# microsoft/tf2-gnn

Measured on NVIDIA H100. Metric: edges/sec (fused gather-msg-scatter), higher is better.
Workload: dtype f32

## Files before the change

### tf2_gnn_b200/csrc/fused_rgcn.cu

```cuda
#include <cuda.h>

#include <algorithm>
#include <cstdio>
#include <cstdlib>
#include <mutex>
#include <vector>

#include "gemm.cuh"
#include "wgmma_tile.cuh"

namespace tfgnn {

constexpr int kFuBM = 128;
constexpr int kFuBK = 32;
constexpr int kFuATileBytes = kFuBM * kFuBK * 4;
constexpr int kFuGatherWarps = 8;
constexpr int kFuFirstGatherWarp = 9;
constexpr int kFuThreads = 32 * (kFuFirstGatherWarp + kFuGatherWarps);
constexpr int kFuMaxSlots = 8;
constexpr int kFuMaxBN = 64;
constexpr int kFuSmemLimit = 227 * 1024;
constexpr int kFuMaxQ = 8;

struct FusedParams {
// ... 90 lines not shown
    ids = ids0B;
    in_blk = 0;
    i_blk = i_pos;
    ids_next = load_ids(i_blk + 32);
    ids0B = load_ids(__shfl_sync(0xffffffffu, rpB, 0));
  }
  template <int NV, int QT = 0, bool FULL = false>
  __device__ __forceinline__ void issue() {
    const int Qc = QT > 0 ? QT : Q;
    while (i_pos == i_end && ic + 1 < ncalls) next_call();
    if (i_pos < i_end) {
      if (in_blk == 32) {
        in_blk = 0;
        i_blk += 32;
        ids = ids_next;
        ids_next = load_ids(i_blk + 32);
      }
      const int s = __shfl_sync(0xffffffffu, ids, in_blk);
      const float* rowp = h + (long long)s * ldh;
#pragma unroll
      for (int j = 0; j < NV; ++j)
        if (FULL || lane + 32 * j < C4) ptx::cp_async16(ibuf + 512u * j, rowp + 128 * j);
      ++in_blk;
      ++i_pos;
    }
    ptx::cp_async_commit();
    if (++islot == Qc) {
      islot = 0;
      ibuf = buf_s;
    } else {
      ibuf += row_bytes;
    }
  }
};

__device__ __forceinline__ void cp_async_wait_oldest(int Q) {
  switch (Q) {
    case 1: asm volatile("cp.async.wait_group 0;" ::: "memory"); break;
    case 2: asm volatile("cp.async.wait_group 1;" ::: "memory"); break;
    case 3: asm volatile("cp.async.wait_group 2;" ::: "memory"); break;
    case 4: asm volatile("cp.async.wait_group 3;" ::: "memory"); break;
    case 5: asm volatile("cp.async.wait_group 4;" ::: "memory"); break;
    case 6: asm volatile("cp.async.wait_group 5;" ::: "memory"); break;
    case 7: asm volatile("cp.async.wait_group 6;" ::: "memory"); break;
    default: asm volatile("cp.async.wait_group 7;" ::: "memory"); break;
  }
}

template <int NV, int QT = 0, bool FULL = false>
__device__ __forceinline__ void gather_warp_main(const FusedParams& p, int lane, int gw, int Q_in, uint8_t* bufs,
                                                 long long unit0, long long unit_step, long long total_units,
                                                 int ctas, int rank, int tile_rows, int row_off, int w_row0, int rpw,
                                                 int ring_row0, uint64_t* slot_ready, uint64_t* slot_free, int split,
                                                 int split_rank, uint32_t peer_slot_ready0) {
  const int Q = QT > 0 ? QT : Q_in;
  const int D = p.D, C4 = p.D >> 2, normalize = p.normalize;
  const bool no_store = p.debug_skip & 16;
  const int kFuSlots = p.num_slots;
  float* const ring = p.ring;
  const uint64_t pol_keep = ptx::policy_evict_last();
  const long long my_units = unit0 < total_units ? (total_units - unit0 + unit_step - 1) / unit_step : 0;
  GatherIssue g;
  g.row_ptr = p.row_ptr; g.src = p.src; g.h = p.h + 4 * lane; g.M = p.M; g.V = p.V; g.L = p.L; g.ldh = p.ldh;
  g.skip = p.debug_skip & 1; g.C4 = C4;
  g.lane = lane; g.gw = gw; g.Q = Q; g.ncalls = (int)(my_units * p.L);
  g.unit0 = unit0; g.unit_step = unit_step; g.ctas = ctas; g.rank = rank;
  g.tile_rows = tile_rows; g.rpw = rpw; g.row_off = row_off; g.w_row0 = w_row0;
  g.buf_s = ptx::smem_u32(bufs) + (uint32_t)lane * 16u;
  g.row_bytes = (uint32_t)p.D * 4;
  g.ic = 0; g.islot = 0; g.in_blk = 0; g.ibuf = g.buf_s;
  g.rpA = g.rp_of(0); g.rpB = g.rp_of(1); g.rpC = g.rp_of(2);
  g.i_pos = __shfl_sync(0xffffffffu, g.rpA, 0);
  g.i_end = __shfl_sync(0xffffffffu, g.rpA, g.nrows_of(0));
  g.i_blk = g.i_pos;
  g.ids = g.load_ids(g.i_blk);
  g.ids_next = g.load_ids(g.i_blk + 32);
  g.ids0B = g.load_ids(__shfl_sync(0xffffffffu, g.rpB, 0));
  int crp = g.rpA, crp_next = g.rpB;
  int cslot = 0;
  uint32_t cbuf = g.buf_s;
  for (int i = 0; i < Q; ++i) g.template issue<NV, QT, FULL>();

  float4 acc[NV];
#pragma unroll
  for (int j = 0; j < NV; ++j) acc[j] = make_float4(0.f, 0.f, 0.f, 0.f);

  for (int cc = 0; cc < g.ncalls; ++cc) {
    int l, v0, nrows;
    g.call_rows(cc, l, v0, nrows);
    const int rp = crp;
    crp = crp_next;
    crp_next = g.rp_of(cc + 2);
    const int slot = cc % kFuSlots;
    if (split) ptx::mbar_wait_cluster(&slot_free[slot], ((cc / kFuSlots) & 1) ^ 1);
    else ptx::mbar_wait_backoff(&slot_free[slot], ((cc / kFuSlots) & 1) ^ 1, p.sleep_long);
    float* dst = ring + ((size_t)ring_row0 + (size_t)slot * tile_rows + (size_t)row_off + (size_t)w_row0) * D + 4 * lane;
    int row = 0;
    int seg_begin = __shfl_sync(0xffffffffu, rp, 0);
    int seg_end = __shfl_sync(0xffffffffu, rp, 1);
    const int e_end = __shfl_sync(0xffffffffu, rp, nrows);
    auto flush = [&]() {
      const float scale = normalize ? 1.0f / ((float)(seg_end - seg_begin) + kSmallNumber) : 1.0f;
#pragma unroll
      for (int j = 0; j < NV; ++j) {
        if (lane + 32 * j < C4 && !no_store)
          ptx::st_f4_hint(dst + 128 * j,
                          make_float4(acc[j].x * scale, acc[j].y * scale, acc[j].z * scale, acc[j].w * scale),
                          pol_keep);
        acc[j] = make_float4(0.f, 0.f, 0.f, 0.f);
      }
      dst += D;
      ++row;
      seg_begin = seg_end;
      seg_end = __shfl_sync(0xffffffffu, rp, row + 1);
    };
    for (int e = seg_begin; e < e_end; ++e) {
      while (e >= seg_end) flush();
      cp_async_wait_oldest(Q);
#pragma unroll
      for (int j = 0; j < NV; ++j) {
        if (FULL || lane + 32 * j < C4) {
          const float4 x = ptx::lds_f4(cbuf + 512u * j);
          acc[j].x += x.x; acc[j].y += x.y; acc[j].z += x.z; acc[j].w += x.w;
        }
      }
      if (++cslot == Q) {
        cslot = 0;
        cbuf = g.buf_s;
      } else {
        cbuf += g.row_bytes;
      }
      g.template issue<NV, QT, FULL>();
    }
    while (row < nrows) flush();
    asm volatile("fence.proxy.async.global;" ::: "memory");
    __syncwarp();
    if (lane == 0) {
      if (split) {
        ptx::mbar_arrive_cluster_release(ptx::mapa_shared(ptx::smem_u32(&slot_ready[slot]), (uint32_t)split_rank));
        ptx::mbar_arrive_cluster_release(peer_slot_ready0 + (uint32_t)slot * 8u);
      } else {
        ptx::mbar_arrive(&slot_ready[slot]);
      }
    }
  }
  asm volatile("cp.async.wait_group 0;" ::: "memory");
}

template <int BN, bool FOLDED = false>
__device__ __forceinline__ void fused_epilogue(const FusedParams& p, const HalfTileAcc<BN>& c, long long m0, int n0, int cw,
                                               int t) {
  const int w = t >> 5, lane = t & 31, cq = 2 * (lane & 3);
  const uint64_t pol_stream = ptx::policy_evict_first();
  const bool ln = p.epi.ln_gamma != nullptr;
#pragma unroll
  for (int h = 0; h < 2; ++h) {
    const long long row = m0 + 64 * cw + 16 * w + (lane >> 2) + 8 * h;
    const bool row_ok = row < p.V;
    float v[BN / 4];
    if (FOLDED) {
#pragma unroll
      for (int i = 0; i < BN / 8; ++i) {
        v[2 * i] = c.main[4 * i + 2 * h];
        v[2 * i + 1] = c.main[4 * i + 2 * h + 1];
      }
    } else {
      acc_row<BN>(c, h, v);
    }
    if (p.epi.row_norm && row_ok) {
      const float inv_rn = 1.0f / fu_row_norm(p.epi, row);
#pragma unroll
      for (int j = 0; j < BN / 4; ++j) v[j] *= inv_rn;
    }
    if (p.epi.bias) {
#pragma unroll
      for (int i = 0; i < BN / 8; ++i) {
        const float2 b = __ldg(reinterpret_cast<const float2*>(p.epi.bias + n0 + 8 * i + cq));
        v[2 * i] += b.x; v[2 * i + 1] += b.y;
      }
    }
    apply_act_vec<BN / 4>(v, p.epi.act);
    if (ln) {
      float s1 = 0.f;
#pragma unroll
      for (int j = 0; j < BN / 4; ++j) s1 += v[j];
      s1 += __shfl_xor_sync(0xffffffffu, s1, 1);
      s1 += __shfl_xor_sync(0xffffffffu, s1, 2);
      const float mean = s1 / (float)BN;
      float s2 = 0.f;
#pragma unroll
      for (int j = 0; j < BN / 4; ++j) { const float d = v[j] - mean; s2 = fmaf(d, d, s2); }
      s2 += __shfl_xor_sync(0xffffffffu, s2, 1);
      s2 += __shfl_xor_sync(0xffffffffu, s2, 2);
      const float rstd = rsqrtf(s2 / (float)BN + p.epi.ln_eps);
#pragma unroll
      for (int i = 0; i < BN / 8; ++i) {
        const float2 g = __ldg(reinterpret_cast<const float2*>(p.epi.ln_gamma + n0 + 8 * i + cq));
        const float2 b = __ldg(reinterpret_cast<const float2*>(p.epi.ln_beta + n0 + 8 * i + cq));
        v[2 * i] = (v[2 * i] - mean) * rstd * g.x + b.x;
        v[2 * i + 1] = (v[2 * i + 1] - mean) * rstd * g.y + b.y;
      }
    }
    if (!row_ok) continue;
#pragma unroll
    for (int i = 0; i < BN / 8; ++i) {
      const long long off = row * p.ldc + n0 + 8 * i + cq;
      const float2 val = make_float2(v[2 * i], v[2 * i + 1]);
      if (p.C_mc) {
        asm volatile("multimem.st.relaxed.sys.global.v2.f32 [%0], {%1, %2};" ::"l"(p.C_mc + off), "f"(val.x), "f"(val.y)
                     : "memory");
      } else {
        asm volatile("st.global.L2::cache_hint.v2.f32 [%0], {%1, %2}, %3;" ::"l"(p.C + off), "f"(val.x), "f"(val.y),
                     "l"(pol_stream)
                     : "memory");
        for (int pr = 0; pr < p.n_peer; ++pr) *reinterpret_cast<float2*>(p.C_peer[pr] + off) = val;
      }
    }
  }
}

template <int NV, int BN>
__global__ void __launch_bounds__(kFuThreads, 1)
fused_rgcn_kernel(const __grid_constant__ CUtensorMap map_a, const __grid_constant__ CUtensorMap map_b,
                  const FusedParams p) {
  extern __shared__ uint8_t smem_raw[];
  uint8_t* smem = reinterpret_cast<uint8_t*>((reinterpret_cast<uintptr_t>(smem_raw) + 1023) & ~uintptr_t(1023));
  constexpr int b_tile_bytes = BN * kFuBK * 4;
  constexpr int stage_bytes = 2 * kFuATileBytes + 2 * b_tile_bytes;
  const int S = p.num_stages;
  const bool split = p.split != 0;
  uint64_t* bars = reinterpret_cast<uint64_t*>(smem + (size_t)S * stage_bytes);
  uint64_t* full = bars;
  uint64_t* empty = bars + S;
  uint64_t* slot_ready = bars + 2 * S;
  uint64_t* slot_free = bars + 2 * S + kFuMaxSlots;
  uint8_t* gbuf = reinterpret_cast<uint8_t*>(
      (reinterpret_cast<uintptr_t>(bars + 2 * S + 2 * kFuMaxSlots) + 127) & ~uintptr_t(127));

  const int warp = threadIdx.x >> 5, lane = threadIdx.x & 31, wg = warp >> 2;
  const uint32_t srank = split ? ptx::cluster_ctarank() : 0u;
  const int kClu = split ? 2 : 1;
  const long long total_units = p.m_tiles;
  const long long unit0 = blockIdx.x / kClu, unit_step = gridDim.x / kClu;
  const int n_pass = p.n_tiles;
  const int kFuSlots = p.num_slots;

  if (threadIdx.x == 0) {
    ptx::prefetch_tensormap(&map_a);
    ptx::prefetch_tensormap(&map_b);
    for (int s = 0; s < S; ++s) {
      ptx::mbar_init(&full[s], 1);
      ptx::mbar_init(&empty[s], 2);
    }
    for (int r = 0; r < kFuMaxSlots; ++r) {
      ptx::mbar_init(&slot_ready[r], kFuGatherWarps * (split ? 2 : 1));
      ptx::mbar_init(&slot_free[r], 2 * (split ? 2 : 1));
    }
    ptx::fence_barrier_init();
  }
  __syncthreads();
  if (split) ptx::cluster_sync_all();
  const int ring_row0 = (split ? blockIdx.x / 2 : blockIdx.x) * kFuSlots * kFuBM;
  const uint32_t peer_slot_ready0 = split ? ptx::mapa_shared(ptx::smem_u32(&slot_ready[0]), srank ^ 1u) : 0u;
  const uint32_t peer_slot_free0 = split ? ptx::mapa_shared(ptx::smem_u32(&slot_free[0]), srank ^ 1u) : 0u;

  if (warp == 8) {
    if (lane == 0) {
      uint32_t it = 0, slot_it = 0;
      const uint64_t pol_keep = ptx::policy_evict_last();
      for (long long unit = unit0; unit < total_units; unit += unit_step, slot_it += p.L) {
        for (int pass = 0; pass < n_pass; ++pass) {
          const int n0 = (int)srank * p.cta_n + pass * BN;
          for (int l = 0; l < p.L; ++l) {
            const uint32_t sq = slot_it + l;
            const int slot = sq % kFuSlots;
            if (split) ptx::mbar_wait_cluster(&slot_ready[slot], (sq / kFuSlots) & 1);
            else ptx::mbar_wait_backoff(&slot_ready[slot], (sq / kFuSlots) & 1, p.sleep_long);
            for (int kb = 0; kb < p.kb_per_type; ++kb, ++it) {
              const int s = it % S;
              const uint32_t ph = (it / S) & 1;
              ptx::mbar_wait_backoff(&empty[s], ph ^ 1, p.sleep_crit);
              uint8_t* st = smem + (size_t)s * stage_bytes;
              ptx::mbar_arrive_expect_tx(&full[s], kFuATileBytes + 2 * b_tile_bytes);
              ptx::tma_load_2d_hint(st, &map_a, &full[s], kb * kFuBK, ring_row0 + slot * kFuBM, pol_keep);
              const int kcol = (l * p.kb_per_type + kb) * kFuBK;
              ptx::tma_load_2d_hint(st + 2 * kFuATileBytes, &map_b, &full[s], kcol, n0, pol_keep);
              ptx::tma_load_2d_hint(st + 2 * kFuATileBytes + b_tile_bytes, &map_b, &full[s], kcol, p.N + n0, pol_keep);
            }
          }
        }
      }
    }
  } else if (wg < 2) {
    const int cw = wg, t = threadIdx.x & 127;
    HalfTileAcc<BN> c;
    uint32_t it = 0, slot_base_it = 0;
    for (long long unit = unit0; unit < total_units; unit += unit_step, slot_base_it += p.L) {
      for (int pass = 0; pass < n_pass; ++pass) {
        int prev_s = 0;
        bool first = true;
        for (int l = 0; l < p.L; ++l) {
          const uint32_t slot_it = slot_base_it + l;
          for (int kb = 0; kb < p.kb_per_type; ++kb, ++it) {
            const int s = it % S;
            const uint32_t ph = (it / S) & 1;
            ptx::mbar_wait_backoff(&full[s], ph, p.sleep_crit);
            const bool slot_done = kb == p.kb_per_type - 1 && pass == n_pass - 1;
            if (slot_done && p.discard_ring && !split) {
              const char* sb = reinterpret_cast<const char*>(
                  p.ring + ((size_t)ring_row0 + (size_t)(slot_it % kFuSlots) * kFuBM + (size_t)cw * 64) * p.D);
              const int lines = 64 * p.D * 4 / 128;
              for (int i = t; i < lines; i += 128) ptx::discard_l2_128(sb + (size_t)i * 128);
            }
            const uint32_t st = ptx::smem_u32(smem + (size_t)s * stage_bytes);
            split_a_half<128>(st, cw, t, p.corr_bf16);
            ptx::fence_proxy_async_smem();
            ptx::warpgroup_sync(1 + cw);
            if (slot_done && t == 0) {
              ptx::mbar_arrive(&slot_free[slot_it % kFuSlots]);
              if (split) ptx::mbar_arrive_cluster_release(peer_slot_free0 + (uint32_t)(slot_it % kFuSlots) * 8u);
            }
            ptx::wgmma_fence();
            mma_kblock<BN, 128>(c, st, st + 2 * kFuATileBytes, cw, p.corr_bf16, first);
            ptx::wgmma_commit();
            ptx::wgmma_wait<1>();
            if (!first && t == 0) ptx::mbar_arrive(&empty[prev_s]);
            prev_s = s;
            first = false;
          }
        }
        ptx::wgmma_wait<0>();
        fence_acc<BN>(c);
        if (t == 0) ptx::mbar_arrive(&empty[prev_s]);
        fused_epilogue<BN>(p, c, unit * kFuBM, (int)srank * p.cta_n + pass * BN, cw, t);
      }
    }
  } else {
    const int gw = warp - kFuFirstGatherWarp;
    uint8_t* my_bufs = gbuf + (size_t)gw * p.gather_q * ((size_t)p.D * 4);
    const int rpw = split ? kFuBM / 2 / kFuGatherWarps : kFuBM / kFuGatherWarps;
    const int row_off = split ? (int)srank * (kFuBM / 2) : 0;
#define TFGNN_FU_GATHER(QT, FULL)                                                                                     \
    gather_warp_main<NV, QT, FULL>(p, lane, gw, p.gather_q, my_bufs, unit0, unit_step, total_units, 1, 0, kFuBM,       \
                                   row_off, gw * rpw, rpw, ring_row0, slot_ready, slot_free, split ? 1 : 0, (int)srank, \
                                   peer_slot_ready0)
    if (p.gather_q == kFuMaxQ && p.D == 128 * NV) TFGNN_FU_GATHER(kFuMaxQ, true);
    else TFGNN_FU_GATHER(0, false);
#undef TFGNN_FU_GATHER
  }

  if (split) {
    __syncwarp();
    ptx::cluster_sync_all();
  }
}

constexpr int kRtBM = 64;
constexpr int kRtATileBytes = kRtBM * kFuBK * 4;
constexpr int kRtGatherWarps = 7;
constexpr int kRtFirstGatherWarp = 9;
constexpr int kRtThreads = 512;
constexpr int kRtMaxH = 256;
constexpr uint32_t kRtConsumerRegs = 184;
constexpr uint32_t kRtOtherRegs = 72;

template <int NV, int BN>
__global__ void __launch_bounds__(kRtThreads, 1)
fused_rgcn_rows_kernel(const __grid_constant__ CUtensorMap map_a, const __grid_constant__ CUtensorMap map_b,
                       const FusedParams p) {
  extern __shared__ uint8_t smem_raw[];
  uint8_t* smem = reinterpret_cast<uint8_t*>((reinterpret_cast<uintptr_t>(smem_raw) + 1023) & ~uintptr_t(1023));
  constexpr int H = 2 * BN;
  constexpr int w_tile_bytes = H * kFuBK * 4;
  constexpr int stage_bytes = 2 * kRtATileBytes + 2 * w_tile_bytes;
  const int S = p.num_stages;
  uint64_t* bars = reinterpret_cast<uint64_t*>(smem + (size_t)S * stage_bytes);
  uint64_t* full = bars;
  uint64_t* empty = bars + S;
  uint64_t* slot_ready = bars + 2 * S;
  uint64_t* slot_free = bars + 2 * S + kFuMaxSlots;
  uint8_t* gbuf = reinterpret_cast<uint8_t*>(
      (reinterpret_cast<uintptr_t>(bars + 2 * S + 2 * kFuMaxSlots) + 127) & ~uintptr_t(127));

  const int warp = threadIdx.x >> 5, lane = threadIdx.x & 31, wg = warp >> 2;
  const uint32_t srank = ptx::cluster_ctarank();
  const long long total_units = (p.m_tiles + 1) / 2;
  const long long unit0 = blockIdx.x / 2, unit_step = gridDim.x / 2;
  const int kSlots = p.num_slots;

  if (threadIdx.x == 0) {
    ptx::prefetch_tensormap(&map_a);
    ptx::prefetch_tensormap(&map_b);
    for (int s = 0; s < S; ++s) {
      ptx::mbar_init(&full[s], 1);
      ptx::mbar_init(&empty[s], 4);
    }
    for (int r = 0; r < kFuMaxSlots; ++r) {
      ptx::mbar_init(&slot_ready[r], kRtGatherWarps);
      ptx::mbar_init(&slot_free[r], 2);
    }
    ptx::fence_barrier_init();
  }
  __syncthreads();
  ptx::cluster_sync_all();
  const int ring_row0 = blockIdx.x * kSlots * kRtBM;

  if (wg >= 2) {
    ptx::setmaxnreg_dec<kRtOtherRegs>();
    if (warp == 8) {
      if (lane == 0) {
        uint32_t it = 0, slot_it = 0;
        const uint64_t pol_keep = ptx::policy_evict_last();
        for (long long unit = unit0; unit < total_units; unit += unit_step, slot_it += p.L) {
          for (int l = 0; l < p.L; ++l) {
            const uint32_t sq = slot_it + l;
            const int slot = sq % kSlots;
            ptx::mbar_wait_backoff(&slot_ready[slot], (sq / kSlots) & 1, p.sleep_long);
            for (int kb = 0; kb < p.kb_per_type; ++kb, ++it) {
              const int s = it % S;
              const uint32_t ph = (it / S) & 1;
              ptx::mbar_wait_cluster(&empty[s], ph ^ 1);
              uint8_t* st = smem + (size_t)s * stage_bytes;
              ptx::mbar_arrive_expect_tx(&full[s], kRtATileBytes + 2 * w_tile_bytes);
              ptx::tma_load_2d_hint(st, &map_a, &full[s], kb * kFuBK, ring_row0 + slot * kRtBM, pol_keep);
              const int kcol = (l * p.kb_per_type + kb) * kFuBK;
              ptx::tma_load_2d_multicast_hint(st + 2 * kRtATileBytes + (int)srank * w_tile_bytes, &map_b, &full[s], kcol,
                                              (int)srank * H, (uint16_t)0x3, pol_keep);
            }
          }
        }
      }
    } else {
      const int gw = warp - kRtFirstGatherWarp;
      const int w_row0 = kRtBM * gw / kRtGatherWarps, rpw = kRtBM * (gw + 1) / kRtGatherWarps - w_row0;
      uint8_t* my_bufs = gbuf + (size_t)gw * p.gather_q * ((size_t)p.D * 4);
#define TFGNN_RT_GATHER(QT, FULL)                                                                                      \
      gather_warp_main<NV, QT, FULL>(p, lane, gw, p.gather_q, my_bufs, unit0, unit_step, total_units, 2, (int)srank,   \
                                     kRtBM, 0, w_row0, rpw, ring_row0, slot_ready, slot_free, 0, 0, 0u)
      if (p.gather_q == kFuMaxQ && p.D == 128 * NV) TFGNN_RT_GATHER(kFuMaxQ, true);
      else TFGNN_RT_GATHER(0, false);
#undef TFGNN_RT_GATHER
    }
  } else {
    ptx::setmaxnreg_inc<kRtConsumerRegs>();
    const int cw = wg, t = threadIdx.x & 127;
    const uint32_t empty0_cta0 = ptx::mapa_shared(ptx::smem_u32(&empty[0]), 0u);
    const uint32_t empty0_cta1 = ptx::mapa_shared(ptx::smem_u32(&empty[0]), 1u);
    auto release_stage = [&](int s) {
      if (t == 0) {
        ptx::mbar_arrive_cluster_release(empty0_cta0 + (uint32_t)s * 8u);
        ptx::mbar_arrive_cluster_release(empty0_cta1 + (uint32_t)s * 8u);
      }
    };
    HalfTileAcc<BN> c;
    uint32_t it = 0, slot_base_it = 0;
    for (long long unit = unit0; unit < total_units; unit += unit_step, slot_base_it += p.L) {
      bool first = true;
      for (int l = 0; l < p.L; ++l) {
        const int slot = (slot_base_it + l) % kSlots;
        for (int kb = 0; kb < p.kb_per_type; ++kb, ++it) {
          const int s = it % S;
          const uint32_t ph = (it / S) & 1;
          ptx::mbar_wait_backoff(&full[s], ph, p.sleep_crit);
          const bool slot_done = kb == p.kb_per_type - 1;
          if (slot_done && p.discard_ring) {
            const char* sb = reinterpret_cast<const char*>(
                p.ring + ((size_t)ring_row0 + (size_t)slot * kRtBM + (size_t)cw * (kRtBM / 2)) * p.D);
            const int lines = kRtBM / 2 * p.D * 4 / 128;
            for (int i = t; i < lines; i += 128) ptx::discard_l2_128(sb + (size_t)i * 128);
          }
          const uint32_t st = ptx::smem_u32(smem + (size_t)s * stage_bytes);
          split_a_half<128, kRtBM>(st, cw, t, p.corr_bf16);
          ptx::fence_proxy_async_smem();
          ptx::warpgroup_pair_sync(1);
          if (slot_done && t == 0) ptx::mbar_arrive(&slot_free[slot]);
          const uint32_t w = st + 2 * kRtATileBytes + (uint32_t)(cw * BN * 128);
          ptx::wgmma_fence();
          mma_kblock_at<BN, 128>(c, st, st + kRtATileBytes, w, w + w_tile_bytes, p.corr_bf16, first);
          ptx::wgmma_commit();
          ptx::wgmma_wait<0>();
          release_stage(s);
          first = false;
        }
      }
      fence_acc<BN>(c);
#pragma unroll
      for (int j = 0; j < BN / 2; ++j) c.main[j] += c.corr[j];
      fused_epilogue<BN, true>(p, c, (2 * unit + srank) * kRtBM, cw * BN, 0, t);
    }
  }
  __syncwarp();
  ptx::cluster_sync_all();
}

typedef CUresult (*EncodeTiledFn)(CUtensorMap*, CUtensorMapDataType, cuuint32_t, void*, const cuuint64_t*,
                                  const cuuint64_t*, const cuuint32_t*, const cuuint32_t*, CUtensorMapInterleave,
                                  CUtensorMapSwizzle, CUtensorMapL2promotion, CUtensorMapFloatOOBfill);
static EncodeTiledFn fu_encode_fn() {
  static EncodeTiledFn fn = nullptr;
  static std::once_flag once;
  std::call_once(once, [] {
    void* p = nullptr;
    cudaDriverEntryPointQueryResult qres;
    if (cudaGetDriverEntryPoint("cuTensorMapEncodeTiled", &p, cudaEnableDefault, &qres) == cudaSuccess &&
        qres == cudaDriverEntryPointSuccess)
      fn = reinterpret_cast<EncodeTiledFn>(p);
  });
  return fn;
}

static int fused_block_n(int n) {
  for (int bn = kFuMaxBN; bn >= 16; bn -= 16)
    if (n % bn == 0) return bn;
  return 0;
}

bool fused_rgcn_supported(long long V, int L, int D, int H, const float* h, const float* out, int ldo) {
  if (V < 1 || L < 1 || D % 32 != 0 || D > 512 || H % 16 != 0 || H < 16 || H > 512) return false;
  if (fused_block_n(H) < H && L + 1 > kFuMaxSlots) return false;
  if ((reinterpret_cast<uintptr_t>(h) | reinterpret_cast<uintptr_t>(out)) & 15) return false;
  if (ldo % 4 != 0) return false;
  return gemm_tc_supported(V, H, L * D, h, D, out, ldo) && fu_encode_fn() != nullptr;
}

bool fused_rgcn_ln_supported(int H) { return H <= kFuMaxBN; }

static std::mutex g_l2_mu;
static int g_l2_want_mb = -1;
static bool g_l2_set[64] = {};
static size_t g_l2_saved[64] = {};

int set_l2_persist_mb(int mb) {
  std::lock_guard<std::mutex> lock(g_l2_mu);
  g_l2_want_mb = mb;
  for (bool& b : g_l2_set) b = false;
  return 0;
}

static size_t g_l2_effective[64] = {};

static int ensure_l2_persist_carveout(size_t need_bytes) {
  int dev = 0;
  TFGNN_CUDA(cudaGetDevice(&dev));
  if (dev < 0 || dev >= 64) return 0;
  std::lock_guard<std::mutex> lock(g_l2_mu);
  long long want_mb = g_l2_want_mb;
  if (want_mb < 0) {
    static const int env_mb = [] { const char* e = getenv("TFGNN_B200_L2_PERSIST_MB"); return e ? atoi(e) : -1; }();
    want_mb = env_mb;
  }
  size_t want = want_mb >= 0 ? (size_t)want_mb << 20 : std::max((size_t)72 << 20, need_bytes + ((size_t)4 << 20));
  if (g_l2_set[dev] && (want_mb >= 0 || g_l2_effective[dev] >= want)) return 0;
  g_l2_set[dev] = true;
  if (want == 0) return 0;
  int max_persist = 0;
  if (cudaDeviceGetAttribute(&max_persist, cudaDevAttrMaxPersistingL2CacheSize, dev) != cudaSuccess || max_persist <= 0) {
    cudaGetLastError();
    return 0;
  }
  if (want > (size_t)max_persist) want = (size_t)max_persist;
  size_t cur = 0;
  if (cudaDeviceGetLimit(&cur, cudaLimitPersistingL2CacheSize) != cudaSuccess) { cudaGetLastError(); return 0; }
  g_l2_effective[dev] = cur;
  if (cur >= want) {
    if (want == (size_t)max_persist) g_l2_effective[dev] = (size_t)-1;
    return 0;
  }
  if (!g_l2_saved[dev]) g_l2_saved[dev] = cur + 1;
  cudaDeviceSetLimit(cudaLimitPersistingL2CacheSize, want);
  cudaGetLastError();
  g_l2_effective[dev] = want == (size_t)max_persist ? (size_t)-1 : want;
  return 0;
}

void restore_l2_persist_carveout() {
  std::lock_guard<std::mutex> lock(g_l2_mu);
  int cur_dev = 0;
  if (cudaGetDevice(&cur_dev) != cudaSuccess) { cudaGetLastError(); return; }
  for (int d = 0; d < 64; ++d) {
    if (!g_l2_saved[d]) continue;
    if (cudaSetDevice(d) == cudaSuccess) cudaDeviceSetLimit(cudaLimitPersistingL2CacheSize, g_l2_saved[d] - 1);
    g_l2_saved[d] = 0;
    g_l2_set[d] = false;
    g_l2_effective[d] = 0;
  }
  cudaSetDevice(cur_dev);
  cudaGetLastError();
}

constexpr int kFuMaxGrid = 160;
static int fused_num_slots(int L, bool multi_pass, bool rows = false) {
  static const int env_slots = [] { const char* e = getenv("TFGNN_B200_RING_SLOTS"); return e ? atoi(e) : 0; }();
  if (multi_pass) return L + 1;
  return (env_slots >= 2 && env_slots <= kFuMaxSlots) ? env_slots : rows ? 3 : 4;
}
size_t fused_rgcn_ring_bytes(int D, int L, int H) {
  (void)H;
  int slots = fused_num_slots(L, false);
  if (L + 1 <= kFuMaxSlots && L + 1 > slots) slots = L + 1;
  return (size_t)kFuMaxGrid * slots * kFuBM * D * sizeof(float);
}

template <int NV, int BN>
static cudaError_t launch_fused_nv_bn(cudaLaunchConfig_t& cfg, const CUtensorMap& map_a, const CUtensorMap& map_b,
                                      const FusedParams& p) {
  static std::once_flag attr_once;
  static cudaError_t attr_err = cudaSuccess;
  std::call_once(attr_once, [] {
    attr_err = cudaFuncSetAttribute(fused_rgcn_kernel<NV, BN>, cudaFuncAttributeMaxDynamicSharedMemorySize, kFuSmemLimit);
  });
  if (attr_err != cudaSuccess) return attr_err;
  return cudaLaunchKernelEx(&cfg, fused_rgcn_kernel<NV, BN>, map_a, map_b, p);
}

template <int NV>
static cudaError_t launch_fused_nv(cudaLaunchConfig_t& cfg, const CUtensorMap& map_a, const CUtensorMap& map_b,
                                   const FusedParams& p) {
  switch (p.block_n) {
    case 16: return launch_fused_nv_bn<NV, 16>(cfg, map_a, map_b, p);
    case 32: return launch_fused_nv_bn<NV, 32>(cfg, map_a, map_b, p);
    case 48: return launch_fused_nv_bn<NV, 48>(cfg, map_a, map_b, p);
    default: return launch_fused_nv_bn<NV, 64>(cfg, map_a, map_b, p);
  }
}

template <int NV, int BN>
static cudaError_t launch_fused_rows_nv_bn(cudaLaunchConfig_t& cfg, const CUtensorMap& map_a, const CUtensorMap& map_b,
                                           const FusedParams& p, long long units, int max_clusters) {
  static std::mutex mu;
  static cudaError_t attr_err = cudaSuccess;
  static bool attr_set = false;
  static size_t occ_smem = 0;
  static int occ_clusters = 0;
  int clusters = 0;
  {
    std::lock_guard<std::mutex> lock(mu);
    if (!attr_set) {
      attr_err = cudaFuncSetAttribute(fused_rgcn_rows_kernel<NV, BN>, cudaFuncAttributeMaxDynamicSharedMemorySize,
                                      kFuSmemLimit);
      attr_set = true;
    }
    if (attr_err != cudaSuccess) return attr_err;
    if (occ_smem != cfg.dynamicSmemBytes) {
      cfg.gridDim = dim3(2u * (unsigned)max_clusters);
      int n = 0;
      cudaError_t e = cudaOccupancyMaxActiveClusters(&n, fused_rgcn_rows_kernel<NV, BN>, &cfg);
      if (e != cudaSuccess) return e;
      if (n < 1) return cudaErrorInvalidConfiguration;
      occ_smem = cfg.dynamicSmemBytes;
      occ_clusters = n;
    }
    clusters = std::min(occ_clusters, max_clusters);
  }
  if (units < clusters) clusters = (int)units;
  cfg.gridDim = dim3(2u * (unsigned)clusters);
  return cudaLaunchKernelEx(&cfg, fused_rgcn_rows_kernel<NV, BN>, map_a, map_b, p);
}

template <int NV>
static cudaError_t launch_fused_rows_nv(cudaLaunchConfig_t& cfg, const CUtensorMap& map_a, const CUtensorMap& map_b,
                                        const FusedParams& p, long long units, int max_clusters) {
  switch (p.block_n) {
    case 48: return launch_fused_rows_nv_bn<NV, 48>(cfg, map_a, map_b, p, units, max_clusters);
    case 64: return launch_fused_rows_nv_bn<NV, 64>(cfg, map_a, map_b, p, units, max_clusters);
    case 80: return launch_fused_rows_nv_bn<NV, 80>(cfg, map_a, map_b, p, units, max_clusters);
    case 96: return launch_fused_rows_nv_bn<NV, 96>(cfg, map_a, map_b, p, units, max_clusters);
    case 112: return launch_fused_rows_nv_bn<NV, 112>(cfg, map_a, map_b, p, units, max_clusters);
    default: return launch_fused_rows_nv_bn<NV, 128>(cfg, map_a, map_b, p, units, max_clusters);
  }
}

int launch_fused_rgcn(const float* h, int D, const int* row_ptr, const int* src, long long M, int V, int L,
                      int normalize, const float* packedB, int corr_bf16, int H, float* ring, float* out, int ldo,
                      const GemmEpilogue& epi, cudaStream_t st, float* const* peer_out, int n_peer_out, float* mc_out) {
  EncodeTiledFn encode = fu_encode_fn();
  if (!encode) {
    set_error(TFGNN_ERR_CUDA, "cuTensorMapEncodeTiled entry point not available");
    return TFGNN_ERR_CUDA;
  }
  int dev = 0, sms = 0;
  TFGNN_CUDA(cudaGetDevice(&dev));
  TFGNN_CUDA(cudaDeviceGetAttribute(&sms, cudaDevAttrMultiProcessorCount, dev));
  FusedParams p{};
  p.h = h; p.ldh = D; p.row_ptr = row_ptr; p.src = src; p.V = V; p.L = L; p.D = D; p.normalize = normalize;
  p.ring = ring;
  p.M = M;
  static const int discard_env = [] { const char* e = getenv("TFGNN_B200_RING_DISCARD"); return e ? atoi(e) : 1; }();
  p.discard_ring = discard_env;
  static const int dbg_env = [] { const char* e = getenv("TFGNN_B200_DEBUG_SKIP"); return e ? atoi(e) : 0; }();
  p.debug_skip = dbg_env;
  p.corr_bf16 = corr_bf16;
  p.n_peer = 0;
  for (int r = 0; r < n_peer_out && r < TFGNN_MAX_PEERS; ++r) p.C_peer[p.n_peer++] = peer_out[r];
  p.C_mc = mc_out;
  p.N = H;
  p.m_tiles = ((long long)V + kFuBM - 1) / kFuBM;
  if (sms > kFuMaxGrid) sms = kFuMaxGrid;
  const bool want_ln = epi.ln_gamma != nullptr;
  TFGNN_REQUIRE(!want_ln || fused_rgcn_ln_supported(H), "fused LayerNorm needs hidden_dim <= 64 (one N pass)");
  const char* split_str = getenv("TFGNN_B200_FUSED_SPLIT");
  const int split_env = split_str ? atoi(split_str) : 1;
  const bool split = !want_ln && split_env != 0 && 2 * p.m_tiles <= sms && H % 32 == 0 &&
                     (fused_block_n(H / 2) == H / 2 || L + 1 <= kFuMaxSlots);
  const bool rows = !split && !want_ln && H > kFuMaxBN && H <= kRtMaxH && H % 32 == 0;
  p.split = split ? 1 : 0;
  p.cta_n = split ? H / 2 : H;
  p.block_n = rows ? H / 2 : fused_block_n(p.cta_n);
  p.n_tiles = rows ? 1 : p.cta_n / p.block_n;
  p.num_slots = fused_num_slots(L, p.n_tiles > 1, rows);
  const int tile_rows = rows ? kRtBM : kFuBM;
  if (rows) p.m_tiles = ((long long)V + kRtBM - 1) / kRtBM;
  p.C = out; p.ldc = ldo; p.epi = epi;
  {
    const char* sc = getenv("TFGNN_B200_SLEEP_CRIT");
    const char* sl = getenv("TFGNN_B200_SLEEP_LONG");
    p.sleep_crit = sc ? (uint32_t)atoi(sc) : 0u;
    p.sleep_long = sl ? (uint32_t)atoi(sl) : 0u;
  }
  const int grid = rows ? (sms & ~1)
                 : split ? (int)(2 * p.m_tiles < (sms & ~1) ? 2 * p.m_tiles : (sms & ~1)) : (int)(p.m_tiles < sms ? p.m_tiles : sms);
  static const int stage_env = [] { const char* e = getenv("TFGNN_B200_FUSED_STAGES"); return e ? atoi(e) : 0; }();
  const char* q_str = getenv("TFGNN_B200_GATHER_Q");
  const int q_env = q_str ? atoi(q_str) : 0;
  const int fixed_bytes = 2048 + 128 + 1024;
  const int row_bytes = D * 4;
  const int want_q = q_env >= 1 && q_env <= kFuMaxQ ? q_env : kFuMaxQ;
  const int gather_warps = rows ? kRtGatherWarps : kFuGatherWarps;
  const int stage_bytes = rows ? 2 * kRtATileBytes + 2 * H * kFuBK * 4 : 2 * kFuATileBytes + 2 * p.block_n * kFuBK * 4;
  auto q_for = [&](int s_) { return (kFuSmemLimit - fixed_bytes - s_ * stage_bytes) / (gather_warps * row_bytes); };
  int stages = stage_env >= 2 ? stage_env : 4;
  while (stages > 2 && q_for(stages) < want_q) --stages;
  int q = q_for(stages);
  if (q > want_q) q = want_q;
  TFGNN_REQUIRE(q >= 1 && stages >= 2, "fused RGCN: tile does not fit shared memory");
  p.kb_per_type = D / kFuBK;
  if (p.debug_skip & 2) p.kb_per_type = 1;
  p.num_stages = stages;
  p.gather_q = q;

  const int Kp = L * D;
  CUtensorMap map_a, map_b;
  {
    cuuint64_t dims[2] = {(cuuint64_t)D, (cuuint64_t)grid * p.num_slots * tile_rows};
    cuuint64_t strides[1] = {(cuuint64_t)D * sizeof(float)};
    cuuint32_t box[2] = {(cuuint32_t)kFuBK, (cuuint32_t)tile_rows};
    cuuint32_t estr[2] = {1, 1};
    CUresult r = encode(&map_a, CU_TENSOR_MAP_DATA_TYPE_FLOAT32, 2, ring, dims, strides, box, estr,
                        CU_TENSOR_MAP_INTERLEAVE_NONE, CU_TENSOR_MAP_SWIZZLE_128B, CU_TENSOR_MAP_L2_PROMOTION_L2_128B,
                        CU_TENSOR_MAP_FLOAT_OOB_FILL_NONE);
    if (r != CUDA_SUCCESS) {
      set_error(TFGNN_ERR_CUDA, "cuTensorMapEncodeTiled(ring) failed with code " + std::to_string((int)r));
      return TFGNN_ERR_CUDA;
    }
  }
  {
    cuuint64_t dims[2] = {(cuuint64_t)Kp, (cuuint64_t)(2 * H)};
    cuuint64_t strides[1] = {(cuuint64_t)Kp * sizeof(float)};
    cuuint32_t box[2] = {(cuuint32_t)kFuBK, (cuuint32_t)(rows ? H : p.block_n)};
    cuuint32_t estr[2] = {1, 1};
    CUresult r = encode(&map_b, CU_TENSOR_MAP_DATA_TYPE_FLOAT32, 2, const_cast<float*>(packedB), dims, strides, box,
                        estr, CU_TENSOR_MAP_INTERLEAVE_NONE, CU_TENSOR_MAP_SWIZZLE_128B,
                        CU_TENSOR_MAP_L2_PROMOTION_L2_256B, CU_TENSOR_MAP_FLOAT_OOB_FILL_NONE);
    if (r != CUDA_SUCCESS) {
      set_error(TFGNN_ERR_CUDA, "cuTensorMapEncodeTiled(B) failed with code " + std::to_string((int)r));
      return TFGNN_ERR_CUDA;
    }
  }
  const size_t smem_bytes = (size_t)stages * stage_bytes + (2 * stages + 2 * kFuMaxSlots) * sizeof(uint64_t) + 128 +
                            (size_t)gather_warps * q * row_bytes + 1024;
  TFGNN_REQUIRE(smem_bytes <= (size_t)kFuSmemLimit, "fused RGCN: shared memory budget exceeded");
  const int nv = (D + 127) / 128;
  {
    const int rc_l2 = ensure_l2_persist_carveout((size_t)grid * p.num_slots * tile_rows * D * sizeof(float) +
                                                 (size_t)2 * H * L * D * sizeof(float));
    if (rc_l2) return rc_l2;
  }
  cudaLaunchConfig_t cfg{};
  cfg.gridDim = dim3((unsigned)grid);
  cfg.blockDim = dim3(rows ? kRtThreads : kFuThreads);
  cfg.dynamicSmemBytes = smem_bytes;
  cfg.stream = st;
  cudaLaunchAttribute attr[1];
  attr[0].id = cudaLaunchAttributeClusterDimension;
  attr[0].val.clusterDim.x = split || rows ? 2u : 1u;
  attr[0].val.clusterDim.y = 1;
  attr[0].val.clusterDim.z = 1;
  cfg.attrs = attr;
  cfg.numAttrs = 1;
  if (rows) {
    const long long units = (p.m_tiles + 1) / 2;
    switch (nv) {
      case 1: TFGNN_CUDA(launch_fused_rows_nv<1>(cfg, map_a, map_b, p, units, grid / 2)); break;
      case 2: TFGNN_CUDA(launch_fused_rows_nv<2>(cfg, map_a, map_b, p, units, grid / 2)); break;
      case 3: TFGNN_CUDA(launch_fused_rows_nv<3>(cfg, map_a, map_b, p, units, grid / 2)); break;
      default: TFGNN_CUDA(launch_fused_rows_nv<4>(cfg, map_a, map_b, p, units, grid / 2)); break;
    }
    TFGNN_LAUNCH_CHECK();
    return 0;
  }
  switch (nv) {
    case 1: TFGNN_CUDA(launch_fused_nv<1>(cfg, map_a, map_b, p)); break;
    case 2: TFGNN_CUDA(launch_fused_nv<2>(cfg, map_a, map_b, p)); break;
    case 3: TFGNN_CUDA(launch_fused_nv<3>(cfg, map_a, map_b, p)); break;
    default: TFGNN_CUDA(launch_fused_nv<4>(cfg, map_a, map_b, p)); break;
  }
  TFGNN_LAUNCH_CHECK();
  return 0;
}

}
```

### tf2_gnn_b200/csrc/sm90_ptx.cuh

```cuda
#pragma once
#include <cuda.h>
#include <cuda_runtime.h>
#include <stdint.h>

namespace tfgnn {
namespace ptx {

__device__ __forceinline__ uint32_t smem_u32(const void* p) {
  return static_cast<uint32_t>(__cvta_generic_to_shared(p));
}

__device__ __forceinline__ void mbar_init(uint64_t* bar, uint32_t count) {
  asm volatile("mbarrier.init.shared::cta.b64 [%0], %1;" ::"r"(smem_u32(bar)), "r"(count) : "memory");
}
__device__ __forceinline__ void fence_barrier_init() {
  asm volatile("fence.mbarrier_init.release.cluster;" ::: "memory");
}
__device__ __forceinline__ void mbar_arrive_expect_tx(uint64_t* bar, uint32_t bytes) {
  asm volatile("mbarrier.arrive.expect_tx.shared::cta.b64 _, [%0], %1;" ::"r"(smem_u32(bar)), "r"(bytes)
               : "memory");
}
__device__ __forceinline__ void mbar_arrive(uint64_t* bar) {
  asm volatile("mbarrier.arrive.shared::cta.b64 _, [%0];" ::"r"(smem_u32(bar)) : "memory");
}
__device__ __forceinline__ void mbar_wait(uint64_t* bar, uint32_t parity) {
  const uint32_t addr = smem_u32(bar);
  uint32_t done;
  do {
    asm volatile(
        "{\n\t.reg .pred p;\n\t"
        "mbarrier.try_wait.parity.shared::cta.b64 p, [%1], %2;\n\t"
        "selp.u32 %0, 1, 0, p;\n\t}"
        : "=r"(done)
        : "r"(addr), "r"(parity)
        : "memory");
  } while (!done);
}
__device__ __forceinline__ void mbar_wait_backoff(uint64_t* bar, uint32_t parity, uint32_t ns) {
  const uint32_t addr = smem_u32(bar);
  for (;;) {
    uint32_t done;
    asm volatile(
        "{\n\t.reg .pred p;\n\t"
        "mbarrier.try_wait.parity.shared::cta.b64 p, [%1], %2;\n\t"
        "selp.u32 %0, 1, 0, p;\n\t}"
        : "=r"(done)
        : "r"(addr), "r"(parity)
        : "memory");
    if (done) break;
    if (ns) asm volatile("nanosleep.u32 %0;" ::"r"(ns));
  }
}

__device__ __forceinline__ void fence_proxy_async_smem() {
  asm volatile("fence.proxy.async.shared::cta;" ::: "memory");
}

__device__ __forceinline__ void prefetch_tensormap(const CUtensorMap* m) {
  asm volatile("prefetch.tensormap [%0];" ::"l"(reinterpret_cast<uint64_t>(m)) : "memory");
}
__device__ __forceinline__ void tma_load_2d(void* smem_dst, const CUtensorMap* map, uint64_t* bar, int c0, int c1) {
  asm volatile(
      "cp.async.bulk.tensor.2d.shared::cluster.global.mbarrier::complete_tx::bytes [%0], [%1, {%3, %4}], [%2];"
      ::"r"(smem_u32(smem_dst)), "l"(reinterpret_cast<uint64_t>(map)), "r"(smem_u32(bar)), "r"(c0), "r"(c1)
      : "memory");
}

__device__ __forceinline__ void tma_prefetch_2d(const CUtensorMap* map, int c0, int c1) {
  asm volatile("cp.async.bulk.prefetch.tensor.2d.L2.global.tile [%0, {%1, %2}];" ::"l"(reinterpret_cast<uint64_t>(map)),
               "r"(c0), "r"(c1)
               : "memory");
}

__device__ __forceinline__ void tma_load_2d_hint(void* smem_dst, const CUtensorMap* map, uint64_t* bar, int c0,
                                                 int c1, uint64_t policy) {
  asm volatile(
      "cp.async.bulk.tensor.2d.shared::cluster.global.mbarrier::complete_tx::bytes.L2::cache_hint"
      " [%0], [%1, {%3, %4}], [%2], %5;"
      ::"r"(smem_u32(smem_dst)), "l"(reinterpret_cast<uint64_t>(map)), "r"(smem_u32(bar)), "r"(c0), "r"(c1),
        "l"(policy)
      : "memory");
}

__device__ __forceinline__ void tma_load_2d_multicast_hint(void* smem_dst, const CUtensorMap* map, uint64_t* bar, int c0,
                                                           int c1, uint16_t cta_mask, uint64_t policy) {
  asm volatile(
      "cp.async.bulk.tensor.2d.shared::cluster.global.mbarrier::complete_tx::bytes.multicast::cluster.L2::cache_hint"
      " [%0], [%1, {%3, %4}], [%2], %5, %6;"
      ::"r"(smem_u32(smem_dst)), "l"(reinterpret_cast<uint64_t>(map)), "r"(smem_u32(bar)), "r"(c0), "r"(c1),
        "h"(cta_mask), "l"(policy)
      : "memory");
}

template <uint32_t REGS>
__device__ __forceinline__ void setmaxnreg_inc() { asm volatile("setmaxnreg.inc.sync.aligned.u32 %0;" ::"n"(REGS)); }
template <uint32_t REGS>
__device__ __forceinline__ void setmaxnreg_dec() { asm volatile("setmaxnreg.dec.sync.aligned.u32 %0;" ::"n"(REGS)); }

__device__ __forceinline__ uint64_t policy_evict_first() {
  uint64_t p;
  asm volatile("createpolicy.fractional.L2::evict_first.b64 %0, 1.0;" : "=l"(p));
  return p;
}
__device__ __forceinline__ uint64_t policy_evict_last() {
  uint64_t p;
  asm volatile("createpolicy.fractional.L2::evict_last.b64 %0, 1.0;" : "=l"(p));
  return p;
}
__device__ __forceinline__ void discard_l2_128(const void* ptr) {
  asm volatile("discard.global.L2 [%0], 128;" ::"l"(ptr) : "memory");
}
__device__ __forceinline__ void cp_async16(uint32_t smem_addr, const void* gptr) {
  asm volatile("cp.async.cg.shared.global [%0], [%1], 16;" ::"r"(smem_addr), "l"(gptr) : "memory");
}
__device__ __forceinline__ void cp_async_commit() { asm volatile("cp.async.commit_group;" ::: "memory"); }
__device__ __forceinline__ void sts_f4(uint32_t saddr, float4 v) {
  asm volatile("st.shared.v4.f32 [%0], {%1,%2,%3,%4};" ::"r"(saddr), "f"(v.x), "f"(v.y), "f"(v.z), "f"(v.w) : "memory");
}
__device__ __forceinline__ void sts_u4(uint32_t saddr, uint4 v) {
  asm volatile("st.shared.v4.b32 [%0], {%1,%2,%3,%4};" ::"r"(saddr), "r"(v.x), "r"(v.y), "r"(v.z), "r"(v.w) : "memory");
}
__device__ __forceinline__ float4 lds_f4(uint32_t saddr) {
  float4 v;
  asm volatile("ld.shared.v4.f32 {%0,%1,%2,%3}, [%4];" : "=f"(v.x), "=f"(v.y), "=f"(v.z), "=f"(v.w) : "r"(saddr) : "memory");
  return v;
}
__device__ __forceinline__ void st_f4_hint(float* ptr, float4 v, uint64_t policy) {
  asm volatile("st.global.L2::cache_hint.v4.f32 [%0], {%1, %2, %3, %4}, %5;" ::"l"(ptr), "f"(v.x), "f"(v.y),
               "f"(v.z), "f"(v.w), "l"(policy)
               : "memory");
}

__device__ __forceinline__ void wgmma_fence() { asm volatile("wgmma.fence.sync.aligned;" ::: "memory"); }
__device__ __forceinline__ void wgmma_commit() { asm volatile("wgmma.commit_group.sync.aligned;" ::: "memory"); }
template <int N>
__device__ __forceinline__ void wgmma_wait() { asm volatile("wgmma.wait_group.sync.aligned %0;" ::"n"(N) : "memory"); }
__device__ __forceinline__ void reg_fence(float& x) { asm volatile("" : "+f"(x)::"memory"); }
__device__ __forceinline__ void warpgroup_sync(int id) { asm volatile("bar.sync %0, 128;" ::"r"(id) : "memory"); }
__device__ __forceinline__ void warpgroup_pair_sync(int id) { asm volatile("bar.sync %0, 256;" ::"r"(id) : "memory"); }

template <int ROW_BYTES>
__device__ __forceinline__ uint64_t gmma_desc_k(uint32_t smem_addr) {
  uint64_t d = 0;
  d |= (uint64_t)((smem_addr >> 4) & 0x3FFF);
  d |= (uint64_t)1 << 16;
  d |= (uint64_t)((8 * ROW_BYTES) >> 4) << 32;
  d |= (uint64_t)(ROW_BYTES == 128 ? 1 : 2) << 62;
  return d;
}

__device__ __forceinline__ uint32_t cluster_ctarank() {
  uint32_t r;
  asm volatile("mov.u32 %0, %%cluster_ctarank;" : "=r"(r));
  return r;
}
__device__ __forceinline__ void cluster_sync_all() {
  asm volatile("barrier.cluster.arrive.release.aligned;\n\tbarrier.cluster.wait.acquire.aligned;" ::: "memory");
}
__device__ __forceinline__ uint32_t mapa_shared(uint32_t local, uint32_t rank) {
  uint32_t r;
  asm volatile("mapa.shared::cluster.u32 %0, %1, %2;" : "=r"(r) : "r"(local), "r"(rank));
  return r;
}
__device__ __forceinline__ void mbar_arrive_cluster(uint32_t cluster_addr) {
  asm volatile("mbarrier.arrive.shared::cluster.b64 _, [%0];" ::"r"(cluster_addr) : "memory");
}
__device__ __forceinline__ void mbar_arrive_cluster_release(uint32_t cluster_addr) {
  asm volatile("mbarrier.arrive.release.cluster.shared::cluster.b64 _, [%0];" ::"r"(cluster_addr) : "memory");
}
__device__ __forceinline__ void mbar_wait_cluster(uint64_t* bar, uint32_t parity) {
  const uint32_t addr = smem_u32(bar);
  uint32_t done;
  do {
    asm volatile(
        "{\n\t.reg .pred p;\n\t"
        "mbarrier.try_wait.parity.acquire.cluster.shared::cta.b64 p, [%1], %2;\n\t"
        "selp.u32 %0, 1, 0, p;\n\t}"
        : "=r"(done)
        : "r"(addr), "r"(parity)
        : "memory");
  } while (!done);
}
__device__ __forceinline__ uint32_t pack_bf16x2(float upper, float lower) {
  uint32_t d;
  asm("cvt.rn.bf16x2.f32 %0, %1, %2;" : "=r"(d) : "f"(upper), "f"(lower));
  return d;
}
__host__ __device__ __forceinline__ float tf32_hi(float x) {
#ifdef __CUDA_ARCH__
  return __uint_as_float(__float_as_uint(x) & 0xFFFFE000u);
#else
  union { float f; uint32_t u; } c; c.f = x; c.u &= 0xFFFFE000u; return c.f;
#endif
}

}
}
```

### tf2_gnn_b200/csrc/wgmma_tile.cuh

```cuda
#pragma once
#include "sm90_ptx.cuh"
#include "wgmma_ops.cuh"

namespace tfgnn {

template <int BN>
struct HalfTileAcc {
  float main[BN / 2];
  float corr[BN / 2];
};

template <int ROW_BYTES, int TILE_ROWS = 128>
__device__ __forceinline__ void split_a_half(uint32_t a_tile, int wg, int t, int corr_bf16) {
  const uint32_t a_s = a_tile + (uint32_t)(wg * (TILE_ROWS / 2) * ROW_BYTES) + (uint32_t)t * 16u;
  const uint32_t lo_s = a_s + (uint32_t)(TILE_ROWS * ROW_BYTES);
  constexpr int kIt = TILE_ROWS / 2 * ROW_BYTES / 16 / 128;
  float4 xs[kIt];
#pragma unroll
  for (int i = 0; i < kIt; ++i) xs[i] = ptx::lds_f4(a_s + (uint32_t)i * 2048u);
#pragma unroll
  for (int i = 0; i < kIt; ++i) {
    const float4 x = xs[i];
    float4 h;
    h.x = ptx::tf32_hi(x.x); h.y = ptx::tf32_hi(x.y); h.z = ptx::tf32_hi(x.z); h.w = ptx::tf32_hi(x.w);
    ptx::sts_f4(a_s + (uint32_t)i * 2048u, h);
    if (corr_bf16) {
      uint4 w;
      w.x = ptx::pack_bf16x2(x.x - h.x, x.x); w.y = ptx::pack_bf16x2(x.y - h.y, x.y);
      w.z = ptx::pack_bf16x2(x.z - h.z, x.z); w.w = ptx::pack_bf16x2(x.w - h.w, x.w);
      ptx::sts_u4(lo_s + (uint32_t)i * 2048u, w);
    } else {
      float4 l;
      l.x = ptx::tf32_hi(x.x - h.x); l.y = ptx::tf32_hi(x.y - h.y);
      l.z = ptx::tf32_hi(x.z - h.z); l.w = ptx::tf32_hi(x.w - h.w);
      ptx::sts_f4(lo_s + (uint32_t)i * 2048u, l);
    }
  }
}

template <int BN, int ROW_BYTES>
__device__ __forceinline__ void mma_kblock_at(HalfTileAcc<BN>& c, uint32_t a_hi, uint32_t a_lo, uint32_t b_hi, uint32_t b_lo,
                                              int corr_bf16, bool first) {
  const uint64_t da_hi = ptx::gmma_desc_k<ROW_BYTES>(a_hi);
  const uint64_t da_lo = ptx::gmma_desc_k<ROW_BYTES>(a_lo);
  const uint64_t db_hi = ptx::gmma_desc_k<ROW_BYTES>(b_hi);
  const uint64_t db_lo = ptx::gmma_desc_k<ROW_BYTES>(b_lo);
#pragma unroll
  for (int k = 0; k < ROW_BYTES / 32; ++k) {
    const uint64_t adv = (uint64_t)(k * 32 >> 4);
    const int acc = (first && k == 0) ? 0 : 1;
    if (corr_bf16) {
      ptx::wgmma_bf16<BN>(c.corr, da_lo + adv, db_lo + adv, acc);
    } else {
      ptx::wgmma_tf32<BN>(c.corr, da_lo + adv, db_hi + adv, acc);
      ptx::wgmma_tf32<BN>(c.corr, da_hi + adv, db_lo + adv, 1);
    }
    ptx::wgmma_tf32<BN>(c.main, da_hi + adv, db_hi + adv, acc);
  }
}
template <int BN, int ROW_BYTES>
__device__ __forceinline__ void mma_kblock(HalfTileAcc<BN>& c, uint32_t a_tile, uint32_t b_tile, int wg, int corr_bf16,
                                           bool first) {
  const uint32_t a_hi = a_tile + (uint32_t)(wg * 64 * ROW_BYTES);
  mma_kblock_at<BN, ROW_BYTES>(c, a_hi, a_hi + 128u * ROW_BYTES, b_tile, b_tile + (uint32_t)(BN * ROW_BYTES), corr_bf16,
                               first);
}

template <int BN>
__device__ __forceinline__ void fence_acc(HalfTileAcc<BN>& c) {
#pragma unroll
  for (int j = 0; j < BN / 2; ++j) {
    ptx::reg_fence(c.main[j]);
    ptx::reg_fence(c.corr[j]);
  }
}

template <int BN>
__device__ __forceinline__ void acc_row(const HalfTileAcc<BN>& c, int h, float (&v)[BN / 4]) {
#pragma unroll
  for (int i = 0; i < BN / 8; ++i) {
    v[2 * i] = c.main[4 * i + 2 * h] + c.corr[4 * i + 2 * h];
    v[2 * i + 1] = c.main[4 * i + 2 * h + 1] + c.corr[4 * i + 2 * h + 1];
  }
}

}
```

Baseline: 1.657 billion.

## Multicast gathered A tile across cluster pair, load per-CTA weight slices

The rows kernel now multicasts each CTA's 64-row half of a 128-row gathered A tile to both CTAs in the cluster, instead of multicasting the full weight tile. Each CTA loads only its own BN-column slice of the hi and lo weights, and each consumer warpgroup synchronises with a 128-thread barrier instead of a pair barrier. This trades duplicated weight traffic for shared activation traffic and changes the output tiling to split columns across the pair. Layer norm is also disabled on the folded epilogue path.

Result: faster. 1.766 billion (median of 6 runs) (+6.6%).

```diff
diff --git a/tf2_gnn_b200/csrc/fused_rgcn.cu b/tf2_gnn_b200/csrc/fused_rgcn.cu
--- a/tf2_gnn_b200/csrc/fused_rgcn.cu
+++ b/tf2_gnn_b200/csrc/fused_rgcn.cu
@@ -266,7 +266,7 @@
                                                int t) {
   const int w = t >> 5, lane = t & 31, cq = 2 * (lane & 3);
   const uint64_t pol_stream = ptx::policy_evict_first();
-  const bool ln = p.epi.ln_gamma != nullptr;
+  const bool ln = !FOLDED && p.epi.ln_gamma != nullptr;
 #pragma unroll
   for (int h = 0; h < 2; ++h) {
     const long long row = m0 + 64 * cw + 16 * w + (lane >> 2) + 8 * h;
@@ -485,8 +485,8 @@
   extern __shared__ uint8_t smem_raw[];
   uint8_t* smem = reinterpret_cast<uint8_t*>((reinterpret_cast<uintptr_t>(smem_raw) + 1023) & ~uintptr_t(1023));
   constexpr int H = 2 * BN;
-  constexpr int w_tile_bytes = H * kFuBK * 4;
-  constexpr int stage_bytes = 2 * kRtATileBytes + 2 * w_tile_bytes;
+  constexpr int b_tile_bytes = BN * kFuBK * 4;
+  constexpr int stage_bytes = 2 * kFuATileBytes + 2 * b_tile_bytes;
   const int S = p.num_stages;
   uint64_t* bars = reinterpret_cast<uint64_t*>(smem + (size_t)S * stage_bytes);
   uint64_t* full = bars;
@@ -535,11 +535,13 @@
               const uint32_t ph = (it / S) & 1;
               ptx::mbar_wait_cluster(&empty[s], ph ^ 1);
               uint8_t* st = smem + (size_t)s * stage_bytes;
-              ptx::mbar_arrive_expect_tx(&full[s], kRtATileBytes + 2 * w_tile_bytes);
-              ptx::tma_load_2d_hint(st, &map_a, &full[s], kb * kFuBK, ring_row0 + slot * kRtBM, pol_keep);
+              ptx::mbar_arrive_expect_tx(&full[s], kFuATileBytes + 2 * b_tile_bytes);
+              ptx::tma_load_2d_multicast_hint(st + (int)srank * kRtATileBytes, &map_a, &full[s], kb * kFuBK,
+                                              ring_row0 + slot * kRtBM, (uint16_t)0x3, pol_keep);
               const int kcol = (l * p.kb_per_type + kb) * kFuBK;
-              ptx::tma_load_2d_multicast_hint(st + 2 * kRtATileBytes + (int)srank * w_tile_bytes, &map_b, &full[s], kcol,
-                                              (int)srank * H, (uint16_t)0x3, pol_keep);
+              ptx::tma_load_2d_hint(st + 2 * kFuATileBytes, &map_b, &full[s], kcol, (int)srank * BN, pol_keep);
+              ptx::tma_load_2d_hint(st + 2 * kFuATileBytes + b_tile_bytes, &map_b, &full[s], kcol, H + (int)srank * BN,
+                                    pol_keep);
             }
           }
         }
@@ -584,13 +586,12 @@
             for (int i = t; i < lines; i += 128) ptx::discard_l2_128(sb + (size_t)i * 128);
           }
           const uint32_t st = ptx::smem_u32(smem + (size_t)s * stage_bytes);
-          split_a_half<128, kRtBM>(st, cw, t, p.corr_bf16);
+          split_a_half<128>(st, cw, t, p.corr_bf16);
           ptx::fence_proxy_async_smem();
-          ptx::warpgroup_pair_sync(1);
+          ptx::warpgroup_sync(1 + cw);
           if (slot_done && t == 0) ptx::mbar_arrive(&slot_free[slot]);
-          const uint32_t w = st + 2 * kRtATileBytes + (uint32_t)(cw * BN * 128);
           ptx::wgmma_fence();
-          mma_kblock_at<BN, 128>(c, st, st + kRtATileBytes, w, w + w_tile_bytes, p.corr_bf16, first);
+          mma_kblock<BN, 128>(c, st, st + 2 * kFuATileBytes, cw, p.corr_bf16, first);
           ptx::wgmma_commit();
           ptx::wgmma_wait<0>();
           release_stage(s);
@@ -600,7 +601,7 @@
       fence_acc<BN>(c);
 #pragma unroll
       for (int j = 0; j < BN / 2; ++j) c.main[j] += c.corr[j];
-      fused_epilogue<BN, true>(p, c, (2 * unit + srank) * kRtBM, cw * BN, 0, t);
+      fused_epilogue<BN, true>(p, c, unit * kFuBM + 64 * cw, (int)srank * BN, 0, t);
     }
   }
   __syncwarp();
@@ -840,7 +841,7 @@
   const int row_bytes = D * 4;
   const int want_q = q_env >= 1 && q_env <= kFuMaxQ ? q_env : kFuMaxQ;
   const int gather_warps = rows ? kRtGatherWarps : kFuGatherWarps;
-  const int stage_bytes = rows ? 2 * kRtATileBytes + 2 * H * kFuBK * 4 : 2 * kFuATileBytes + 2 * p.block_n * kFuBK * 4;
+  const int stage_bytes = 2 * kFuATileBytes + 2 * p.block_n * kFuBK * 4;
   auto q_for = [&](int s_) { return (kFuSmemLimit - fixed_bytes - s_ * stage_bytes) / (gather_warps * row_bytes); };
   int stages = stage_env >= 2 ? stage_env : 4;
   while (stages > 2 && q_for(stages) < want_q) --stages;
@@ -870,7 +871,7 @@
   {
     cuuint64_t dims[2] = {(cuuint64_t)Kp, (cuuint64_t)(2 * H)};
     cuuint64_t strides[1] = {(cuuint64_t)Kp * sizeof(float)};
-    cuuint32_t box[2] = {(cuuint32_t)kFuBK, (cuuint32_t)(rows ? H : p.block_n)};
+    cuuint32_t box[2] = {(cuuint32_t)kFuBK, (cuuint32_t)p.block_n};
     cuuint32_t estr[2] = {1, 1};
     CUresult r = encode(&map_b, CU_TENSOR_MAP_DATA_TYPE_FLOAT32, 2, const_cast<float*>(packedB), dims, strides, box,
                         estr, CU_TENSOR_MAP_INTERLEAVE_NONE, CU_TENSOR_MAP_SWIZZLE_128B,
diff --git a/tf2_gnn_b200/csrc/sm90_ptx.cuh b/tf2_gnn_b200/csrc/sm90_ptx.cuh
--- a/tf2_gnn_b200/csrc/sm90_ptx.cuh
+++ b/tf2_gnn_b200/csrc/sm90_ptx.cuh
@@ -137,7 +137,6 @@
 __device__ __forceinline__ void wgmma_wait() { asm volatile("wgmma.wait_group.sync.aligned %0;" ::"n"(N) : "memory"); }
 __device__ __forceinline__ void reg_fence(float& x) { asm volatile("" : "+f"(x)::"memory"); }
 __device__ __forceinline__ void warpgroup_sync(int id) { asm volatile("bar.sync %0, 128;" ::"r"(id) : "memory"); }
-__device__ __forceinline__ void warpgroup_pair_sync(int id) { asm volatile("bar.sync %0, 256;" ::"r"(id) : "memory"); }
 
 template <int ROW_BYTES>
 __device__ __forceinline__ uint64_t gmma_desc_k(uint32_t smem_addr) {
diff --git a/tf2_gnn_b200/csrc/wgmma_tile.cuh b/tf2_gnn_b200/csrc/wgmma_tile.cuh
--- a/tf2_gnn_b200/csrc/wgmma_tile.cuh
+++ b/tf2_gnn_b200/csrc/wgmma_tile.cuh
@@ -10,11 +10,11 @@
   float corr[BN / 2];
 };
 
-template <int ROW_BYTES, int TILE_ROWS = 128>
+template <int ROW_BYTES>
 __device__ __forceinline__ void split_a_half(uint32_t a_tile, int wg, int t, int corr_bf16) {
-  const uint32_t a_s = a_tile + (uint32_t)(wg * (TILE_ROWS / 2) * ROW_BYTES) + (uint32_t)t * 16u;
-  const uint32_t lo_s = a_s + (uint32_t)(TILE_ROWS * ROW_BYTES);
-  constexpr int kIt = TILE_ROWS / 2 * ROW_BYTES / 16 / 128;
+  const uint32_t a_s = a_tile + (uint32_t)(wg * 64 * ROW_BYTES) + (uint32_t)t * 16u;
+  const uint32_t lo_s = a_s + 128u * ROW_BYTES;
+  constexpr int kIt = 64 * ROW_BYTES / 16 / 128;
   float4 xs[kIt];
 #pragma unroll
   for (int i = 0; i < kIt; ++i) xs[i] = ptx::lds_f4(a_s + (uint32_t)i * 2048u);
@@ -39,12 +39,13 @@
 }
 
 template <int BN, int ROW_BYTES>
-__device__ __forceinline__ void mma_kblock_at(HalfTileAcc<BN>& c, uint32_t a_hi, uint32_t a_lo, uint32_t b_hi, uint32_t b_lo,
-                                              int corr_bf16, bool first) {
+__device__ __forceinline__ void mma_kblock(HalfTileAcc<BN>& c, uint32_t a_tile, uint32_t b_tile, int wg, int corr_bf16,
+                                           bool first) {
+  const uint32_t a_hi = a_tile + (uint32_t)(wg * 64 * ROW_BYTES);
   const uint64_t da_hi = ptx::gmma_desc_k<ROW_BYTES>(a_hi);
-  const uint64_t da_lo = ptx::gmma_desc_k<ROW_BYTES>(a_lo);
-  const uint64_t db_hi = ptx::gmma_desc_k<ROW_BYTES>(b_hi);
-  const uint64_t db_lo = ptx::gmma_desc_k<ROW_BYTES>(b_lo);
+  const uint64_t da_lo = ptx::gmma_desc_k<ROW_BYTES>(a_hi + 128u * ROW_BYTES);
+  const uint64_t db_hi = ptx::gmma_desc_k<ROW_BYTES>(b_tile);
+  const uint64_t db_lo = ptx::gmma_desc_k<ROW_BYTES>(b_tile + (uint32_t)(BN * ROW_BYTES));
 #pragma unroll
   for (int k = 0; k < ROW_BYTES / 32; ++k) {
     const uint64_t adv = (uint64_t)(k * 32 >> 4);
@@ -57,13 +58,6 @@
     }
     ptx::wgmma_tf32<BN>(c.main, da_hi + adv, db_hi + adv, acc);
   }
-}
-template <int BN, int ROW_BYTES>
-__device__ __forceinline__ void mma_kblock(HalfTileAcc<BN>& c, uint32_t a_tile, uint32_t b_tile, int wg, int corr_bf16,
-                                           bool first) {
-  const uint32_t a_hi = a_tile + (uint32_t)(wg * 64 * ROW_BYTES);
-  mma_kblock_at<BN, ROW_BYTES>(c, a_hi, a_hi + 128u * ROW_BYTES, b_tile, b_tile + (uint32_t)(BN * ROW_BYTES), corr_bf16,
-                               first);
 }
 
 template <int BN>
```
